# SmallVCM/SmallVCM

Hardware: AMD Instinct MI355X
Metric: Mpaths/sec (light+camera), VCM scene 1 at 2048^2 (higher is better)
Workload: dtype f32; 1 GPU; scene 1 -a vcm 2048x2048 maxPathLength 10 minPathLength 0 radiusFactor 0.003 radiusAlpha 0.75 seed 1234, iterations 5..408 timed; parallelism=1 renderer(s) (iteration-parallel, smallvcm.cxx:61-108) on one GPU, 1 in flight

## Files before the change

### smallvcm_amd/csrc/vcm_api.hip

```cpp
#include <hip/hip_runtime.h>
#include <stdio.h>
#include <stdlib.h>
#include <string.h>
#include <string>
#include <new>
#include <mutex>
#include <vector>
#include <condition_variable>
#include <atomic>

#include "vcm_kernels.h"
#include "vcm_kat.h"
#include "scene_host.h"
#include "scene_kind.h"
#include "vcm_denoise.h"
#include "vcm_variance.h"
#include "vcm_robust.h"
#include "vcm_parts.h"
#include "vcm_display.h"

using namespace vcm;

static thread_local std::string g_err;
static int fail(const char *what, const char *detail)
// ... 70 lines not shown
    Arena *arenas[VCM_MAX_ARENAS];
};
static std::atomic<unsigned long long> g_threadCounter{0};
static thread_local unsigned long long g_threadId = 0;
static unsigned long long this_thread_id() { if (!g_threadId) g_threadId = ++g_threadCounter; return g_threadId; }

#ifndef VCM_MERGE_DEFAULT
#define VCM_MERGE_DEFAULT VCM_MERGE_PAIRS
#endif
struct vcm_ctx : Scratch {
    SceneHost *scene;
    bool useVM, useVC, lightTraceOnly, ppm;
    int renderer;
    float baseRadius, radiusAlpha;
    int seed, device, rank, world;
    int resX, resY, N, p0, nLocal;
    int iterations;

    hipStream_t stream;
    bool ownStream;
    hipStream_t side;
    hipEvent_t evFork, evBbox, evGrid;
    bool gridInFlight;
    hipStream_t splat;
    hipEvent_t evSplatFork, evSplatDone;
    hipEvent_t evSortFork, evSorted;
    hipEvent_t evZero;
    bool prezeroed, sortInFlight;
    bool splatInFlight;
    bool resolveInFlight;
    hipEvent_t evMergeDone, evSplatWork, evResolved;
    hipEvent_t evPreMerge;
    bool mergeInFlight;
    bool deviceReady;
    ArenaPool *pool;
    Arena *arena; bool holdsArena;

    DScene *dScene;
    char *dSceneBlob;
    float *dFb;
    unsigned char *dRngLight, *dRngCam;
    GridHeader *dHdr;
    unsigned long long *dStats;
    unsigned long long *dStatsRing;
    unsigned long long *dStamps;
    float radiusRing[VCM_STAMP_RING];
// ... 240 lines not shown
}
static void arena_release(vcm_ctx *c, bool recordEvent)
{
    if (!c->holdsArena) return;
    Arena *a = c->arena;
    const bool recorded = recordEvent && a->eventReady && hipEventRecord(a->lastUse, c->resolveInFlight ? c->splat : c->stream) == hipSuccess;
    c->holdsArena = false;
    {
        std::lock_guard<std::mutex> g(*a->mtx);
        if (recorded) { a->lastValid = true; a->lastUser = c; }
        a->busy = false;
        a->ownerThread = 0;
    }
    a->cv->notify_all();
}
static int abort_iteration(vcm_ctx *c, int rc)
{
    if (rc != 0 && c && c->inIteration && c->holdsArena) {
        const std::string keep = g_err;
        (void)hipStreamSynchronize(c->stream);
        if (c->deviceReady) { (void)hipStreamSynchronize(c->side); (void)hipStreamSynchronize(c->splat); }
        c->mergeInFlight = false;
        c->gridInFlight = false;
        c->splatInFlight = false;
        c->resolveInFlight = false;
        c->sortInFlight = false;
        c->inIteration = false;
        arena_release(c, false);
        g_err = keep;
    } else if (rc != 0 && c && c->holdsArena && !c->inIteration) {
        arena_release(c, false);
    }
    return rc;
}

static int scratch_readable(vcm_ctx *c, const char *what)
{
    if (!c || !c->deviceReady || (!c->inIteration && c->iterations == 0)) return fail(what, "no iteration has run");
    if (!c->holdsArena) {
        if (!c->arena) return fail(what, "no iteration has run");
        std::lock_guard<std::mutex> g(*c->arena->mtx);
        if (c->arena->lastUser != c)
            return fail(what, "the iteration scratch has since been used by another context of this device");
    }
    return 0;
}
// ... 179 lines not shown
    hipLaunchKernelGGL((k_scan_apply<T>), dim3(nTiles), dim3(VCM_SCAN_BLOCK), 0, stream, in, n, (const int *)tileSums, out, totalOut, writeTotalAtN);
    HIPCHK(hipGetLastError());
    return 0;
}
template <typename T>
static int launch_scan(vcm_ctx *c, const T *in, int n, int *out, int *totalOut, int writeTotalAtN)
{
    return launch_scan_on<T>(c, 0, c->stream, in, n, out, totalOut, writeTotalAtN, take_stamps(c, c->stream));
}

static int shape_knob(const char *key)
{
    static const char *spec = getenv("SMALLVCM_AMD_SHAPE");
    if (!spec) return 0;
    const size_t n = strlen(key);
    for (const char *p = spec; *p;) {
        if (!strncmp(p, key, n) && p[n] == '=') { const int v = atoi(p + n + 1); return v > 0 ? v : 0; }
        const char *q = strchr(p, ',');
        if (!q) break;
        p = q + 1;
    }
    return 0;
}
static void trace_launch_shape(int nLocal, int *blocks, int *chunk, bool lightPass = false)
{
    int waves = (nLocal + VCM_WAVE - 1) / VCM_WAVE;
    const int tw = shape_knob("trace_waves");
    int maxWaves = tw ? tw : 256 * 16;
    if (!tw && nLocal <= (1 << 20)) maxWaves = 256 * 12;
    const int lw = shape_knob("light_waves");
    if (lightPass && lw) maxWaves = lw;
    if (maxWaves > VCM_MAX_TRACE_WAVES) maxWaves = VCM_MAX_TRACE_WAVES;
    if (waves > maxWaves) waves = maxWaves;
    if (waves < 1) waves = 1;
    const int wavesPerBlock = VCM_TRACE_BLOCK / VCM_WAVE;
    *blocks = (waves + wavesPerBlock - 1) / wavesPerBlock;
    const int totalWaves = *blocks * wavesPerBlock;
    int ch = nLocal / totalWaves;
    const int ce = shape_knob("trace_chunk");
    if (ce) ch = ce;
    if (!ce && !tw && nLocal <= (1 << 20)) {
        ch = 128;
        const int need = (nLocal + ch - 1) / ch;
        if (totalWaves > need) *blocks = (need + wavesPerBlock - 1) / wavesPerBlock;
    }
    *chunk = ch < 64 ? 64 : (ch > 256 && !ce ? 256 : ch);
}


template <class Launch>
static int read_back(vcm_ctx *c, const char *who, size_t bytes, void *host, Launch &&launch)
{
// ... 381 lines not shown
    P.wavefront = vcm_is_wavefront(c, maxLen);
    P.renderer = c->renderer;
    P.iteration = iteration;
    const bool big = c->nLocal >= (1 << 20);
    P.qblockVertex = big ? 512 : 256; P.qblockDI = big ? 512 : 256; P.qblockVC = big ? 1024 : 512;
    {
        const int perPath = shape_knob("buckets_per_path");
        const int per = perPath ? perPath : (c->nLocal > (1 << 20) ? 16 : 4);
        long long nb = (long long)per * c->nLocal;
        if (nb < (1 << 18)) nb = 1 << 18;
        P.nBuckets = nb < VCM_QSORT_BUCKETS ? (int)nb : VCM_QSORT_BUCKETS;
    }
    P.foreignOut = 0;

    c->nPend[0] = c->nPend[1] = 0;
    if (mark(c, EV_START)) return -1;
    c->dStats = c->dStatsRing + (size_t)(c->iterations % VCM_STAMP_RING) * VCM_STAT_SLOTS;
    c->radiusRing[c->iterations % VCM_STAMP_RING] = radius;
    if (zero_ranges(c->stream, c->dStats, VCM_STAT_SLOTS * sizeof(unsigned long long), c->store.count, (size_t)c->nLocal ,
                    c->vs.count, 32 * sizeof(int) ,
                    c->dHdr, 6 * sizeof(uint32_t) )) return -1;
    c->importedRecords = false;
    c->importedSorted = false;
    c->gridBuilt = c->cameraTraced = c->merged = c->splatsPending = c->recordsValid = c->countedInCamera = c->scatteredInDI = c->gridInFlight = c->splatInFlight = c->bboxPreset = c->bboxFromLight = c->bboxFinal = c->prezeroed = c->sortInFlight = c->spaceSet = c->mergeImported = false;
    c->splatInFlight = c->resolveInFlight;
    c->inIteration = true;
    c->lastMergeKernel = 0;
    c->evValid = false;
    return 0;
}

static int task_blocks(int nLocal)
{
    const int n = shape_knob("task_blocks");
    if (n) return n;
    if (nLocal >= (1 << 21)) return 256 * 12;
    const int b = nLocal / 1024;
    return b < 512 ? 512 : (b > 1024 ? 1024 : b);
}
static int merge_blocks(int nLocal, int N)
{
    const int n = shape_knob("merge_blocks") >= 8 ? (shape_knob("merge_blocks") & ~7) : 0;
    if (n) return n;
    if (nLocal >= (1 << 21)) return 16384;
    int b = (nLocal / 1024) & ~7;
    b = b < 512 ? 512 : (b > 2048 ? 2048 : b);
    if (N >= (1 << 21) && nLocal < N) { const long long d = (16384ll * nLocal / N) & ~7ll; if (d > b) b = (int)d; }
// ... 112 lines not shown
        launch_kind<kWrapLens | kWrapPick | kWrapSobol | kWrapGgx>(c, [&](auto tag) {
            using S = typename decltype(tag)::type;
            hipLaunchKernelGGL((k_light_trace<0, S>), dim3(blocks), dim3(VCM_TRACE_BLOCK), 0, c->stream, c->dScene, c->P, c->store,
                               c->dFb, c->dRngLight, c->dStats, chunk, take_stamps(c, c->stream), c->vs.count + 16, c->dHdr);
        });
    HIPCHK(hipGetLastError());
    c->bboxFromLight = c->world == 1;
    if (mark(c, EV_LIGHT_K1)) return -1;
    if (launch_scan<unsigned char>(c, c->store.count, c->nLocal, c->dPathStart, c->dLocalTotal, 0)) return -1;
    if (c->mergeInFlight) { HIPCHK(hipStreamWaitEvent(c->stream, c->evMergeDone, 0)); c->mergeInFlight = false; }
    bool countsSet = false;
    if (c->useVM || wf) {
        c->recordsValid = c->useVM && c->world > 1 && !c->sortedExchange;
        const bool fold = c->world == 1;
        hipLaunchKernelGGL((c->ggx ? k_compact_records_ggx : k_compact_records), dim3(aux_blocks(c->nLocal)), dim3(256), 0, c->stream, (const DScene *)c->dScene, c->P, c->store, c->dPathStart,
                           c->dRecordsLocal, c->dSlotOfVertex, c->recordsValid ? 1 : 0, fold ? c->dHdr : (GridHeader *)NULL,
                           (const int *)c->dLocalTotal, (fold && c->bboxFromLight) ? 1 : 0);
        HIPCHK(hipGetLastError());
        countsSet = fold;
        if (fold && c->bboxFromLight) c->bboxFinal = true;
    }
    if (wf && (c->useVC || c->lightTraceOnly)) {
        c->splatsPending = true;
        if (c->world == 1 && flush_light_splats(c)) return -1;
    }
    if (mark(c, EV_LIGHT)) return -1;
    if (!countsSet) {
        hipLaunchKernelGGL(k_set_counts, dim3(1), dim3(1), 0, c->stream, c->dHdr, c->dLocalTotal, 1, 0, take_stamps(c, c->stream));
        HIPCHK(hipGetLastError());
    }
    return 0;
}

static int ensure_records(vcm_ctx *c)
{
    if (c->recordsValid || !c->useVM) return 0;
    hipLaunchKernelGGL((c->ggx ? k_compact_records_ggx : k_compact_records), dim3(aux_blocks(c->nLocal)), dim3(256), 0, c->stream, (const DScene *)c->dScene, c->P, c->store, c->dPathStart,
                       c->dRecordsLocal, c->dSlotOfVertex, 1, (GridHeader *)NULL, (const int *)c->dLocalTotal, 0);
    HIPCHK(hipGetLastError());
    c->recordsValid = true;
    return 0;
}

int vcm_light_records(vcm_ctx *c, void **devPtr, long long *count)
{
    if (scratch_readable(c, "vcm_light_records")) return -1;
    if (use_device(c)) return -1;
// ... 78 lines not shown

static int vcm_import_light_records_impl(vcm_ctx *c, const void *devPtr, const long long *counts, int nSeg, long long strideRecords)
{
    if (!c || !c->inIteration) return fail("vcm_import_light_records", "no iteration in progress");
    if (c->world <= 1 || !c->dRecordsAll) return fail("vcm_import_light_records", "context is not sharded");
    if (use_device(c)) return -1;
    long long total = 0;
    const size_t recBytes = VCM_MERGE_RECORD_FLOATS * sizeof(float);
    for (int s = 0; s < nSeg; s++) {
        if (counts[s] < 0) return fail("vcm_import_light_records", "negative count");
        if (total + counts[s] > (long long)c->arena->capS * (long long)c->arena->capN) return fail("vcm_import_light_records", "too many records");
        if (counts[s] > 0)
            HIPCHK(hipMemcpyAsync((char *)c->dRecordsAll + (size_t)total * recBytes,
                                  (const char *)devPtr + (size_t)s * (size_t)strideRecords * recBytes,
                                  (size_t)counts[s] * recBytes, hipMemcpyDeviceToDevice, c->stream));
        total += counts[s];
    }
    hipLaunchKernelGGL(k_set_counts, dim3(1), dim3(1), 0, c->stream, c->dHdr, c->dLocalTotal, 0, (int)total, take_stamps(c, c->stream));
    HIPCHK(hipGetLastError());
    c->importedRecords = true;
    return 0;
}

static const I2 *sort_cells_radix(vcm_ctx *c, hipStream_t q, int scanSlot, const VertexSource &recs)
{
    const int nCells = c->P.nCells;
    int bits = 1;
    while (bits < 31 && (1ll << bits) < (long long)nCells) bits++;
    const int passes = (bits + 7) / 8;
    const int V = radix_sort_blocks(c->nLocal);
    static_assert(256 * VCM_RSORT_MAX_BLOCKS <= VCM_QSORT_BUCKETS, "the scan scratch (dTileSums) is sized for the bucket table: the digit matrix must not be larger");
    const StampArgs none = { { NULL, NULL, NULL, NULL } };
    uint32_t *key[2] = { (uint32_t *)c->dCellId, (uint32_t *)c->dSortedIndex };
    I2 *pay[2] = { (I2 *)c->dUnsorted, (I2 *)c->dUnsorted + (size_t)c->arena->capS * c->arena->capN };
    int *hist = c->dRadixHist, *scanned = c->dRadixHist + 256 * VCM_RSORT_MAX_BLOCKS;
    hipLaunchKernelGGL(k_cell_keys, dim3(V), dim3(256), 0, q, c->P, recs, (const GridHeader *)c->dHdr, key[0], pay[0], hist, take_stamps(c, q));
    int cur = 0;
    for (int p = 0; p < passes; p++) {
        if (p > 0) hipLaunchKernelGGL(k_radix_hist, dim3(V), dim3(256), 0, q, (const uint32_t *)key[cur], (const GridHeader *)c->dHdr, 8 * p, hist);
        if (hipGetLastError() != hipSuccess) { fail("vcm_build_grid", "radix histogram launch"); return NULL; }
        if (launch_scan_on<int>(c, scanSlot, q, hist, 256 * V, scanned, NULL, 0, none)) return NULL;
        hipLaunchKernelGGL(k_radix_scatter, dim3(V), dim3(256), 0, q, (const uint32_t *)key[cur], (const I2 *)pay[cur], key[cur ^ 1], pay[cur ^ 1],
                           (const GridHeader *)c->dHdr, 8 * p, (const int *)scanned);
        cur ^= 1;
    }
    hipLaunchKernelGGL(k_cell_starts, dim3(aux_blocks(c->nLocal)), dim3(256), 0, q, (const uint32_t *)key[cur], (const GridHeader *)c->dHdr, nCells, c->dCellStart);
    if (hipGetLastError() != hipSuccess) { fail("vcm_build_grid", "radix sort launch"); return NULL; }
    return pay[cur];
}

static int sorted_shape(vcm_ctx *c, long long strideRecords, int *K, int *nBlocks, long long *slabWords, const char *who)
{
    if (!c) return fail(who, "ctx is NULL");
    if (c->world <= 1) return fail(who, "the context is not sharded");
    if (!c->useVM) return fail(who, "the algorithm does not merge: nothing to exchange");
    if (c->world > VCM_SORTED_MAX_SHARDS) return fail(who, "more than 64 shards: use the unsorted exchange");
    if (strideRecords < 1 || strideRecords >= (1ll << 24)) return fail(who, "1 <= records per shard < 2^24 (the index shares a word with the path length): use the unsorted exchange");
    *K = sorted_block_cells(c->world);
    *nBlocks = (c->N + *K - 1) / *K;
    const long long w = strideRecords * VCM_SORTED_WORDS + (long long)*nBlocks + 1;
    *slabWords = (w + 3) & ~3ll;
    return 0;
}
extern "C" long long vcm_sorted_slab_words(vcm_ctx *c, long long strideRecords)
{
    int K, nBlocks; long long words;
    if (sorted_shape(c, strideRecords, &K, &nBlocks, &words, "vcm_sorted_slab_words")) return -1;
    return words;
}
// ... 40 lines not shown
    long long total = 0;
    for (int s = 0; s < nSeg; s++) {
        if (counts[s] < 0 || counts[s] > strideRecords) return fail("vcm_import_sorted_light_records", "a count exceeds the slab");
        in.rankBase[s] = (int)total;
        total += counts[s];
    }
    in.rankBase[nSeg] = (int)total;
    if (total > (long long)c->arena->capS * (long long)c->arena->capN) return fail("vcm_import_sorted_light_records", "too many records");
    hipLaunchKernelGGL(k_set_counts, dim3(1), dim3(1), 0, c->stream, c->dHdr, c->dLocalTotal, 0, (int)total, take_stamps(c, c->stream));
    HIPCHK(hipGetLastError());
    c->importedSorted = true;
    c->importedRecords = false;
    return 0;
}
extern "C" int vcm_sort_light_records(vcm_ctx *c, void *dstDev, long long strideRecords)
{
    return abort_iteration(c, vcm_sort_light_records_impl(c, dstDev, strideRecords));
}
extern "C" int vcm_import_sorted_light_records(vcm_ctx *c, const void *gathered, const long long *counts, int nSeg, long long strideRecords)
{
    return abort_iteration(c, vcm_import_sorted_light_records_impl(c, gathered, counts, nSeg, strideRecords));
}

static int join_grid(vcm_ctx *c)
{
    if (!c->gridInFlight) return 0;
    HIPCHK(hipStreamWaitEvent(c->stream, c->evGrid, 0));
    c->gridInFlight = false;
    return 0;
}

static int vcm_build_grid_impl(vcm_ctx *c)
{
    if (!c || !c->inIteration) return fail("vcm_build_grid", "no iteration in progress");
    if (use_device(c)) return -1;
    if (flush_light_splats(c)) return -1;
    c->gridBuilt = true;
    if (c->useVM) {
        hipStream_t q = c->side;
        HIPCHK(hipEventRecord(c->evFork, c->stream));
        HIPCHK(hipStreamWaitEvent(q, c->evFork, 0));
        if (mark_on(c, EV_GRID_K0, q)) return -1;
        if (c->importedSorted) {
            if (!c->bboxPreset) return fail("vcm_build_grid", "sorted records without the box they were sorted with");
            const int blocks = c->sortedIn.nBlocks < 8192 ? c->sortedIn.nBlocks : 8192;
            hipLaunchKernelGGL(k_grid_merge_blocks, dim3(blocks), dim3(256), 0, q, c->P, (const GridHeader *)c->dHdr, c->sortedIn, c->dCellStart,
                               c->dGx, c->dGy, c->dGz, c->dGb, c->dG1, c->dG2, c->dG3, c->dSortedIndex, take_stamps(c, q));
            HIPCHK(hipGetLastError());
            if (mark_on(c, EV_GRID, q)) return -1;
            hipLaunchKernelGGL(k_note_grid_vertices, dim3(1), dim3(1), 0, q, (const GridHeader *)c->dHdr, c->dStats + STAT_COUNT, take_stamps(c, q));
            HIPCHK(hipGetLastError());
            HIPCHK(hipEventRecord(c->evGrid, q));
            c->gridInFlight = true;
            if (!c->P.wavefront && join_grid(c)) return -1;
            return 0;
        }
        VertexSource recs;
        recs.records = c->importedRecords ? c->dRecordsAll : (c->recordsValid ? c->dRecordsLocal : NULL);
        recs.store = c->store;
        recs.slotOfVertex = c->dSlotOfVertex;
        const int nCells = c->P.nCells;
        const dim3 g(aux_blocks(c->nLocal)), b(256);
        const bool radix = grid_sort_is_radix(c);
        if (c->prezeroed) HIPCHK(hipStreamWaitEvent(q, c->evZero, 0));
        else if (!radix && zero_ranges(q, c->dCellCount, ((size_t)nCells + 1) * sizeof(int))) return -1;
        bool boxOnSide = false;
        if (!c->bboxPreset) {
            if (c->bboxFromLight && !recs.records) {
                if (!c->bboxFinal) { hipLaunchKernelGGL(k_bbox_finalize, dim3(1), dim3(64), 0, q, c->dHdr, 1); boxOnSide = true; }
            } else {
                boxOnSide = true;
                hipLaunchKernelGGL(k_grid_init, dim3(1), dim3(64), 0, q, c->dHdr, take_stamps(c, q));
                hipLaunchKernelGGL(k_bbox, dim3(512), b, 0, q, recs, c->dHdr);
                hipLaunchKernelGGL(k_bbox_finalize, dim3(1), dim3(64), 0, q, c->dHdr, 0);
            }
        }
        HIPCHK(hipEventRecord(c->evBbox, q));
        const I2 *sorted = NULL;
        if (radix) {
            if (!(sorted = sort_cells_radix(c, q, 1, recs))) return -1;
        } else {
            hipLaunchKernelGGL(k_cell_count, g, b, 0, q, c->P, recs, (const GridHeader *)c->dHdr, c->dCellId,
                               c->dSortedIndex , c->dCellCount, take_stamps(c, q));
            HIPCHK(hipGetLastError());
            if (launch_scan_on<int>(c, 1, q, c->dCellCount, nCells, c->dCellStart, NULL, 1, take_stamps(c, q))) return -1;
            hipLaunchKernelGGL(k_cell_scatter, g, b, 0, q, (const GridHeader *)c->dHdr, (const int *)c->dCellId,
                               (const int *)c->dSortedIndex, (const int *)c->dCellStart,
                               recs.records ? (const int *)NULL : (const int *)c->dSlotOfVertex, c->dUnsorted);
        }
        hipLaunchKernelGGL((c->ggx ? k_cell_rank_gather_ggx : k_cell_rank_gather), g, b, 0, q, (const DScene *)c->dScene, (const GridHeader *)c->dHdr, recs,
                           (const int *)c->dCellStart, (const I4 *)c->dUnsorted, sorted, c->dGx,
                           c->dGy, c->dGz, c->dGb, c->dG1, c->dG2, c->dG3, c->dSortedIndex);
        if (mark_on(c, EV_GRID, q)) return -1;
        hipLaunchKernelGGL(k_note_grid_vertices, dim3(1), dim3(1), 0, q, (const GridHeader *)c->dHdr, c->dStats + STAT_COUNT, take_stamps(c, q));
        HIPCHK(hipGetLastError());
        HIPCHK(hipEventRecord(c->evGrid, q));
        if (boxOnSide) HIPCHK(hipStreamWaitEvent(c->stream, c->evBbox, 0));
        c->gridInFlight = true;
        if (!c->P.wavefront && join_grid(c)) return -1;
    } else {
        if (mark(c, EV_GRID_K0)) return -1;
        if (mark(c, EV_GRID)) return -1;
    }
    return 0;
}

static GridStore grid_of(vcm_ctx *c)
{
    GridStore grid;
    grid.cellStart = c->dCellStart; grid.gx = c->dGx; grid.gy = c->dGy; grid.gz = c->dGz; grid.gb = c->dGb; grid.g1 = c->dG1; grid.g2 = c->dG2; grid.g3 = c->dG3;
    grid.hdr = c->dHdr;
    return grid;
}

static int vcm_trace_camera_impl(vcm_ctx *c)
{
    if (!c || !c->inIteration) return fail("vcm_trace_camera", "no iteration in progress");
    if (use_device(c)) return -1;
    if (flush_light_splats(c)) return -1;
    c->cameraTraced = true;
    if (c->lightTraceOnly) return 0;
    int blocks, chunk;
    trace_launch_shape(c->nLocal, &blocks, &chunk);
    if (c->resolveInFlight) HIPCHK(hipStreamWaitEvent(c->stream, c->evResolved, 0));
    if (mark(c, EV_CAMERA_K0)) return -1;
    if (c->renderer) {
        if (c->renderer == 1)
            launch_kind<kWrapLens | kWrapPick | kWrapSobol | kWrapGgx>(c, [&](auto tag) {
                using S = typename decltype(tag)::type;
                hipLaunchKernelGGL((k_path_trace<S>), dim3(blocks), dim3(VCM_TRACE_BLOCK), 0, c->stream, c->dScene, c->P, c->dCamOut,
                                   c->dRngCam, c->dStats, chunk, take_stamps(c, c->stream), c->vs.count + 8);
            });
        else
            launch_kind<kWrapLens | kWrapSobol>(c, [&](auto tag) {
                using S = typename decltype(tag)::type;
                hipLaunchKernelGGL((k_eye_light<S>), dim3(2048), dim3(256), 0, c->stream, c->dScene, c->P, c->dCamOut, c->dRngCam,
                                   c->dStats, take_stamps(c, c->stream));
            });
        HIPCHK(hipGetLastError());
        if (mark(c, EV_CAMERA_K1)) return -1;
        if (mark(c, EV_CONNECT_K1)) return -1;
        return 0;
    }
    if (c->P.wavefront) {
        c->countedInCamera = c->useVM && (c->gridBuilt || c->bboxPreset);
        c->vs.sortHdr = c->countedInCamera ? c->dHdr : NULL;
// ... 5 lines not shown
            else if (zero_ranges(c->stream, c->dQueryCount, ((size_t)c->P.nBuckets + 1) * sizeof(int))) return -1;
        }
        launch_kind<kWrapLens | kWrapPick | kWrapSobol | kWrapGgx>(c, [&](auto tag) {
            using S = typename decltype(tag)::type;
            hipLaunchKernelGGL((k_camera_trace<1, S>), dim3(blocks), dim3(VCM_TRACE_BLOCK), 0, c->stream, c->dScene, c->P,
                               c->store, grid_of(c), c->vs, c->dCamOut, c->dCamMask, c->dRngCam, c->dStats, chunk, take_stamps(c, c->stream));
        });
        if (mark(c, EV_CAMERA_K1)) return -1;
        if (c->useVC) {
            c->scatteredInDI = c->countedInCamera && c->P.minLen <= 2;
            const bool inlineSort = c->scatteredInDI && (c->nLocal <= (1 << 20) || grid_sort_is_radix(c));
            if (c->countedInCamera && c->world == 1 && !inlineSort) {
                HIPCHK(hipEventRecord(c->evSortFork, c->stream));
                HIPCHK(hipStreamWaitEvent(c->side, c->evSortFork, 0));
                const StampArgs none = { { NULL, NULL, NULL, NULL } };
                if (launch_scan_on<int>(c, 3, c->side, c->dQueryCount, c->P.nBuckets, c->dQueryStart, NULL, 1, none)) return -1;
                hipLaunchKernelGGL(k_query_scatter, dim3(aux_blocks(c->nLocal)), dim3(256), 0, c->side, c->vs, (const int *)c->dQueryKey,
                                   (const int *)c->dQueryArrival, (const int *)c->dQueryStart, c->dSortedVertex);
                HIPCHK(hipEventRecord(c->evSorted, c->side));
                c->sortInFlight = true;
                c->scatteredInDI = false;
            }
            if (c->scatteredInDI && launch_scan<int>(c, c->dQueryCount, c->P.nBuckets, c->dQueryStart, NULL, 1)) return -1;
            {
                HIPCHK(hipEventRecord(c->evSplatFork, c->stream));
                HIPCHK(hipStreamWaitEvent(c->splat, c->evSplatFork, 0));
                launch_kind<kWrapGgx>(c, [&](auto tag) {
                    using S = typename decltype(tag)::type;
                    hipLaunchKernelGGL((k_connect_vc<S>), dim3(task_blocks(c->nLocal)), dim3(VCM_TASK_BLOCK), 0, c->splat, c->dScene, c->P, c->vs,
                                       c->store, c->dStats);
                });
                HIPCHK(hipEventRecord(c->evSplatDone, c->splat));
                c->splatInFlight = true;
            }
            launch_kind<kWrapPick | kWrapSobol | kWrapGgx>(c, [&](auto tag) {
                using S = typename decltype(tag)::type;
                hipLaunchKernelGGL((k_connect_di<S>), dim3(task_blocks(c->nLocal)), dim3(VCM_TASK_BLOCK), 0, c->stream, c->dScene, c->P, c->vs,
                                   c->dStats, c->scatteredInDI ? (const int *)c->dQueryStart : (const int *)NULL,
                                   c->scatteredInDI ? c->dSortedVertex : (int *)NULL, take_stamps(c, c->stream));
            });
        }
        if (mark(c, EV_CONNECT_K1)) return -1;
    } else {
        if (c->useVM && !c->gridBuilt) return fail("vcm_trace_camera", "strict mode merges inside the camera pass: call vcm_build_grid first");
        launch_kind<kWrapLens | kWrapPick | kWrapSobol | kWrapGgx>(c, [&](auto tag) {
            using S = typename decltype(tag)::type;
            hipLaunchKernelGGL((k_camera_trace<0, S>), dim3(blocks), dim3(VCM_TRACE_BLOCK), 0, c->stream, c->dScene, c->P,
                               c->store, grid_of(c), c->vs, c->dCamOut, c->dCamMask, c->dRngCam, c->dStats, chunk, take_stamps(c, c->stream));
        });
        if (mark(c, EV_CAMERA_K1)) return -1;
        if (mark(c, EV_CONNECT_K1)) return -1;
    }
    HIPCHK(hipGetLastError());
    if (c->world > 1 && flush_stamps(c, c->stream)) return -1;
    return 0;
}

#define VCM_SPACE_BLOCKS 512
static int space_scratch(vcm_ctx *c)
{
    if (c->dSpaceMatrix) return 0;
    HIPCHK(hipMalloc((void **)&c->dSpaceMatrix, sizeof(int) * VCM_SPACE_MAX_SLABS * VCM_SPACE_BLOCKS));
    HIPCHK(hipMalloc((void **)&c->dSpaceScanned, sizeof(int) * (VCM_SPACE_MAX_SLABS * VCM_SPACE_BLOCKS + 1)));
    HIPCHK(hipMalloc((void **)&c->dSpaceTotals, sizeof(int) * VCM_SPACE_MAX_SLABS));
    HIPCHK(hipMalloc((void **)&c->dSpaceHist, sizeof(int) * 256));
    return 0;
}
static int space_ready(vcm_ctx *c, const char *who)
{
    if (!c || !c->inIteration) return fail(who, "no iteration in progress");
    if (c->world <= 1) return fail(who, "the context is not sharded");
    if (!c->useVM || !c->P.wavefront) return fail(who, "needs a merging algorithm in wavefront mode");
    if (use_device(c)) return -1;
    return space_scratch(c);
}
static int vcm_space_histogram_impl(vcm_ctx *c, int axis, float *lo, float *binWidth, int *hist256)
// ... 152 lines not shown
    if (!c->lightTraceOnly) {
        bool mergeAside = false;
        if (mark(c, EV_MERGE_K0)) return -1;
        if (c->P.wavefront && c->useVM && c->mergeImported) {
            if (mark(c, EV_SORT_K1)) return -1;
        } else if (c->P.wavefront && c->useVM) {
            if (!c->gridBuilt) return fail("vcm_merge", "call vcm_build_grid first");
            const int nb = c->P.nBuckets;
            if (!c->countedInCamera) {
                if (c->prezeroed) HIPCHK(hipStreamWaitEvent(c->stream, c->evZero, 0));
                if (zero_ranges(c->stream, c->dQueryCount, ((size_t)nb + 1) * sizeof(int))) return -1;
                hipLaunchKernelGGL(k_query_count, dim3(aux_blocks(c->nLocal)), dim3(256), 0, c->stream, c->P, c->vs,
                                   (const GridHeader *)c->dHdr, c->dQueryKey, c->dQueryArrival, c->dQueryCount, take_stamps(c, c->stream));
            }
            if (c->sortInFlight) {
                HIPCHK(hipStreamWaitEvent(c->stream, c->evSorted, 0));
                c->sortInFlight = false;
            } else if (!c->scatteredInDI) {
                if (launch_scan<int>(c, c->dQueryCount, nb, c->dQueryStart, NULL, 1)) return -1;
                hipLaunchKernelGGL(k_query_scatter, dim3(aux_blocks(c->nLocal)), dim3(256), 0, c->stream, c->vs, (const int *)c->dQueryKey,
                                   (const int *)c->dQueryArrival, (const int *)c->dQueryStart, c->dSortedVertex);
            }
            if (mark(c, EV_SORT_K1)) return -1;
            if (c->gridInFlight && hipEventQuery(c->evGrid) != hipSuccess) { (void)hipGetLastError(); if (flush_stamps(c, c->stream)) return -1; }
            if (join_grid(c)) return -1;
            mergeAside = (c->nLocal <= (1 << 20) || !c->useVC) && c->world == 1 && !c->strictOrder;
            hipStream_t ks = c->stream;
            if (mergeAside) {
                if (flush_stamps(c, c->stream)) return -1;
                HIPCHK(hipEventRecord(c->evPreMerge, c->stream));
                HIPCHK(hipStreamWaitEvent(c->side, c->evPreMerge, 0));
                ks = c->side;
            }
            static int mergeChunk = 0;
            if (!mergeChunk) mergeChunk = shape_knob("merge_chunk") ? shape_knob("merge_chunk") : 16;
            int mergeStaged = c->mergeKind;
            if (mergeStaged == VCM_MERGE_PAIRS && (int)c->scene->materials.size() > VCM_PAIR_MATERIALS) mergeStaged = VCM_MERGE_WALK;
            c->lastMergeKernel = mergeStaged;
            hipLaunchKernelGGL(merge_kernel(mergeStaged, c->intPhong, c->ggx), dim3(merge_blocks(c->nLocal, c->N)), dim3(VCM_MERGE_BLOCK), 0, ks, c->dScene, c->P, grid_of(c),
                               c->vs, (const int *)c->dSortedVertex, (const int *)(c->dQueryStart + nb), c->dStats, mergeChunk, take_stamps(c, c->stream));
        } else {
            if (mark(c, EV_SORT_K1)) return -1;
        }
        if (mergeAside) {
            HIPCHK(hipGetLastError());
            HIPCHK(hipEventRecord(c->evMergeDone, c->side));
// ... 1173 lines not shown
```

### smallvcm_amd/csrc/vcm_kernels.h

```cpp
#ifndef SMALLVCM_AMD_VCM_KERNELS_H
#define SMALLVCM_AMD_VCM_KERNELS_H

#include <hip/hip_runtime.h>
#include "vcm_core.h"

namespace vcm {

enum { STAT_LIGHT_RAYS = 0, STAT_CAMERA_RAYS, STAT_SHADOW_RAYS, STAT_MERGE_QUERIES, STAT_MERGE_CANDIDATES,
       STAT_MERGE_ACCEPTED, STAT_CONNECTIONS, STAT_LIGHT_SPLATS, STAT_STORED, STAT_COUNT };

#define VCM_TRACE_BLOCK 256
#define VCM_WAVE 64

struct StampArgs { unsigned long long *p[4]; };
__device__ __forceinline__ void stamp_entry(const StampArgs &s)
{
    if (blockIdx.x == 0 && threadIdx.x == 0 && s.p[0]) {
        const unsigned long long t = wall_clock64();
#pragma unroll
        for (int k = 0; k < 4; k++) if (s.p[k]) *s.p[k] = t;
    }
}

__device__ __forceinline__ unsigned lane_id() { return __builtin_amdgcn_mbcnt_hi(~0u, __builtin_amdgcn_mbcnt_lo(~0u, 0u)); }
// ... 1626 lines not shown
            for (int round = 0; round < VCM_RSORT_TILE / 256; round++) {
                if (validBits & (1u << round)) {
                    const uint32_t d = (k[round] >> shift) & 255u;
                    const int pos = sRun[w][d] + r[round];
                    sKey[pos] = k[round];
                    sPay[pos] = p[round];
                }
            }
            __syncthreads();
            for (int j = tid; j < m; j += 256) {
                const uint32_t kk = sKey[j];
                const uint32_t d = (kk >> shift) & 255u;
                const int dst = sGlobal[d] + (j - sBinStart[d]);
                keyOut[dst] = kk;
                payOut[dst] = sPay[j];
            }
            __syncthreads();
            sGlobal[tid] += total;
        }
    }
#endif
}

__global__ void __launch_bounds__(256) k_cell_starts(const uint32_t *__restrict__ key, const GridHeader *__restrict__ hdr, int nCells, int *cellStart)
{
#if defined(__HIP_DEVICE_COMPILE__)
    const int n = hdr->nRecords;
    const int lane = (int)threadIdx.x & 63;
    const int stride = (int)(gridDim.x * blockDim.x);
    for (int base = (int)(blockIdx.x * blockDim.x) + ((int)threadIdx.x & ~63); base <= n; base += stride) {
        const int pos = base + lane;
        int c0 = 0, len = 0;
        if (pos <= n) {
            const int prev = pos > 0 ? (int)key[pos - 1] : -1;
            const int cur = pos < n ? (int)key[pos] : nCells;
            c0 = prev + 1; len = cur - prev;
        }
        const int head = len < 8 ? len : 8;
        for (int c = 0; c < head; c++) cellStart[c0 + c] = pos;
        unsigned long long longOnes = __ballot(len > 8);
        while (longOnes) {
            const int l = __ffsll((long long)longOnes) - 1;
            longOnes &= longOnes - 1ull;
            const int s = __shfl(c0 + 8, l, 64), e = __shfl(c0 + len, l, 64), v = __shfl(pos, l, 64);
            for (int c = s + lane; c < e; c += 64) cellStart[c] = v;
        }
    }
#endif
}

template <class S>
__device__ __forceinline__ void cell_rank_gather_body(const DScene *__restrict__ scp, const GridHeader *__restrict__ hdr, const VertexSource &src,
                                                      const int *__restrict__ cellStart, const I4 *__restrict__ unsorted, const I2 *__restrict__ sorted,
                                                      float *gx, float *gy, float *gz, float *gb, F4 *g1, F4 *g2, F2 *g3, int *sortedIndex)
{
    const int n = hdr->nRecords;
    for (int pos = blockIdx.x * blockDim.x + threadIdx.x; pos < n; pos += gridDim.x * blockDim.x) {
        I4 me;
        int dst = pos;
        if (sorted) {
            const I2 e = sorted[pos];
            me.x = e.x; me.y = e.y; me.z = 0; me.w = 0;
        } else {
            me = unsorted[pos];
            const int cell = me.z;
            const int lo = cellStart[cell], hi = cellStart[cell + 1];
            int rank = 0;
            for (int q = lo; q < hi; q++) rank += (unsorted[q].x < me.x) ? 1 : 0;
            dst = lo + rank;
        }
        const int i = me.x;
        F2 t;
        if (src.records) {
            const float *r = src.records + (size_t)i * VCM_MERGE_RECORD_FLOATS;
            gx[dst] = r[0]; gy[dst] = r[1]; gz[dst] = r[2];
            gb[grid_blocked_index(dst, 0)] = r[0]; gb[grid_blocked_index(dst, 1)] = r[1]; gb[grid_blocked_index(dst, 2)] = r[2];
            g1[dst] = mk4(r[3], r[4], r[5], r[11]);
            g2[dst] = mk4(r[6], r[7], r[8], r[9]);
            t.x = r[10]; t.y = r[12];
        } else {
            const size_t slot = (size_t)me.y;
            const F4 a = lv(src.store, slot, 0), b = lv(src.store, slot, 1), d = lv(src.store, slot, 3);
            const F4 e = light_vertex_wdir_contprob(*static_cast<const S *>(scp), a, lv(src.store, slot, 2), d, false);
            gx[dst] = a.x; gy[dst] = a.y; gz[dst] = a.z;
            gb[grid_blocked_index(dst, 0)] = a.x; gb[grid_blocked_index(dst, 1)] = a.y; gb[grid_blocked_index(dst, 2)] = a.z;
            g1[dst] = e;
            g2[dst] = b;
            t.x = d.w; t.y = u2f(f2u(a.w) & 0xffu);
        }
        g3[dst] = t;
        if (sortedIndex) sortedIndex[dst] = i;
    }
}
__global__ void __launch_bounds__(256) k_cell_rank_gather(const DScene *__restrict__ scp, const GridHeader *__restrict__ hdr, VertexSource src,
                                   const int *__restrict__ cellStart, const I4 *__restrict__ unsorted, const I2 *__restrict__ sorted,
                                   float *gx, float *gy, float *gz, float *gb, F4 *g1, F4 *g2, F2 *g3, int *sortedIndex)
{
    const int n = hdr->nRecords;
    for (int pos = blockIdx.x * blockDim.x + threadIdx.x; pos < n; pos += gridDim.x * blockDim.x) {
        I4 me;
        int dst = pos;
        if (sorted) {
            const I2 e = sorted[pos];
            me.x = e.x; me.y = e.y; me.z = 0; me.w = 0;
        } else {
            me = unsorted[pos];
            const int cell = me.z;
            const int lo = cellStart[cell], hi = cellStart[cell + 1];
            int rank = 0;
            for (int q = lo; q < hi; q++) rank += (unsorted[q].x < me.x) ? 1 : 0;
            dst = lo + rank;
        }
        const int i = me.x;
        F2 t;
        if (src.records) {
            const float *r = src.records + (size_t)i * VCM_MERGE_RECORD_FLOATS;
            gx[dst] = r[0]; gy[dst] = r[1]; gz[dst] = r[2];
            gb[grid_blocked_index(dst, 0)] = r[0]; gb[grid_blocked_index(dst, 1)] = r[1]; gb[grid_blocked_index(dst, 2)] = r[2];
            g1[dst] = mk4(r[3], r[4], r[5], r[11]);
            g2[dst] = mk4(r[6], r[7], r[8], r[9]);
            t.x = r[10]; t.y = r[12];
        } else {
            const size_t slot = (size_t)me.y;
            const F4 a = lv(src.store, slot, 0), b = lv(src.store, slot, 1), d = lv(src.store, slot, 3);
            const F4 e = light_vertex_wdir_contprob(*scp, a, lv(src.store, slot, 2), d, false);
            gx[dst] = a.x; gy[dst] = a.y; gz[dst] = a.z;
            gb[grid_blocked_index(dst, 0)] = a.x; gb[grid_blocked_index(dst, 1)] = a.y; gb[grid_blocked_index(dst, 2)] = a.z;
            g1[dst] = e;
            g2[dst] = b;
            t.x = d.w; t.y = u2f(f2u(a.w) & 0xffu);
        }
        g3[dst] = t;
        if (sortedIndex) sortedIndex[dst] = i;
    }
}
__global__ void __launch_bounds__(256) k_cell_rank_gather_ggx(const DScene *__restrict__ scp, const GridHeader *__restrict__ hdr, VertexSource src,
                                       const int *__restrict__ cellStart, const I4 *__restrict__ unsorted, const I2 *__restrict__ sorted,
                                       float *gx, float *gy, float *gz, float *gb, F4 *g1, F4 *g2, F2 *g3, int *sortedIndex)
{
    cell_rank_gather_body<WithGgx<DScene>>(scp, hdr, src, cellStart, unsorted, sorted, gx, gy, gz, gb, g1, g2, g3, sortedIndex);
}


#define VCM_SORTED_WORDS 13
#define VCM_SORTED_MAX_SHARDS 64
#define VCM_SORTED_MAX_TABLE 4096
inline __host__ __device__ int sorted_block_cells(int S)
{
    const int k = VCM_SORTED_MAX_TABLE / (S > 0 ? S : 1);
    int p = 16;
    while (p * 2 <= k && p < 1024) p *= 2;
    return p;
}

template <class S>
__device__ __forceinline__ void cell_rank_pack_body(const DScene *__restrict__ scp, const GridHeader *__restrict__ hdr, const VertexSource &src,
                                                    const int *__restrict__ cellStart, const I4 *__restrict__ unsorted, const I2 *__restrict__ sorted,
                                                    uint32_t *slab, int *blockStart, int nCells, int K, int nBlocks)
{
    const int n = hdr->nRecords;
    for (int b = blockIdx.x * blockDim.x + threadIdx.x; b <= nBlocks; b += gridDim.x * blockDim.x) {
        const long long c = (long long)b * K;
        blockStart[b] = cellStart[c < nCells ? (int)c : nCells];
// ... 173 lines not shown
```

Baseline: 1254 Mpaths/s.

## Defer grid gather tail and fuse cell-start computation into rank gather kernel

Adds an 'early plan' for large single-GPU VCM runs. The grid is built before the light splats are flushed, and the final gather/cell-starts step is deferred so it can run on the side stream behind the camera trace. The cell_starts kernel and the note_grid_vertices kernel are fused into the rank-gather kernel, which removes two launches. The camera trace uses fewer waves in this mode to leave room for the overlapped work. The cost is more complex stream ordering and the risk of contention between the overlapped kernels.

```diff
diff --git a/smallvcm_amd/csrc/vcm_api.hip b/smallvcm_amd/csrc/vcm_api.hip
--- a/smallvcm_amd/csrc/vcm_api.hip
+++ b/smallvcm_amd/csrc/vcm_api.hip
@@ -116,6 +116,8 @@
     hipStream_t side;
     hipEvent_t evFork, evBbox, evGrid;
     bool gridInFlight;
+    bool gridTailPending;
+    VertexSource tailRecs; const I2 *tailSorted; const uint32_t *tailKey;
     hipStream_t splat;
     hipEvent_t evSplatFork, evSplatDone;
     hipEvent_t evSortFork, evSorted;
@@ -402,6 +404,7 @@
         if (c->deviceReady) { (void)hipStreamSynchronize(c->side); (void)hipStreamSynchronize(c->splat); }
         c->mergeInFlight = false;
         c->gridInFlight = false;
+        c->gridTailPending = false;
         c->splatInFlight = false;
         c->resolveInFlight = false;
         c->sortInFlight = false;
@@ -627,12 +630,37 @@
     }
     return 0;
 }
-static void trace_launch_shape(int nLocal, int *blocks, int *chunk, bool lightPass = false)
+static bool shape_word(const char *key, const char *word)
+{
+    static const char *spec = getenv("SMALLVCM_AMD_SHAPE");
+    if (!spec) return false;
+    const size_t n = strlen(key), m = strlen(word);
+    for (const char *p = spec; *p;) {
+        if (!strncmp(p, key, n) && p[n] == '=') return !strncmp(p + n + 1, word, m) && (p[n + 1 + m] == ',' || p[n + 1 + m] == 0);
+        const char *q = strchr(p, ',');
+        if (!q) break;
+        p = q + 1;
+    }
+    return false;
+}
+static int plan_forced()
+{
+    static const int f = shape_word("plan", "early") ? 1 : (shape_word("plan", "late") ? 2 : 0);
+    return f;
+}
+static bool plan_early(const vcm_ctx *c)
+{
+    if (c->world != 1 || c->strictOrder) return false;
+    if (plan_forced()) return plan_forced() == 1;
+    return c->useVC && c->useVM && c->nLocal > (1 << 20);
+}
+static void trace_launch_shape(int nLocal, int *blocks, int *chunk, bool lightPass = false, bool early = false)
 {
     int waves = (nLocal + VCM_WAVE - 1) / VCM_WAVE;
     const int tw = shape_knob("trace_waves");
     int maxWaves = tw ? tw : 256 * 16;
     if (!tw && nLocal <= (1 << 20)) maxWaves = 256 * 12;
+    if (!tw && early && !lightPass && nLocal > (1 << 20)) maxWaves = 256 * 12;
     const int lw = shape_knob("light_waves");
     if (lightPass && lw) maxWaves = lw;
     if (maxWaves > VCM_MAX_TRACE_WAVES) maxWaves = VCM_MAX_TRACE_WAVES;
@@ -1060,7 +1088,7 @@
                     c->dHdr, 6 * sizeof(uint32_t) )) return -1;
     c->importedRecords = false;
     c->importedSorted = false;
-    c->gridBuilt = c->cameraTraced = c->merged = c->splatsPending = c->recordsValid = c->countedInCamera = c->scatteredInDI = c->gridInFlight = c->splatInFlight = c->bboxPreset = c->bboxFromLight = c->bboxFinal = c->prezeroed = c->sortInFlight = c->spaceSet = c->mergeImported = false;
+    c->gridBuilt = c->cameraTraced = c->merged = c->splatsPending = c->recordsValid = c->countedInCamera = c->scatteredInDI = c->gridInFlight = c->gridTailPending = c->splatInFlight = c->bboxPreset = c->bboxFromLight = c->bboxFinal = c->prezeroed = c->sortInFlight = c->spaceSet = c->mergeImported = false;
     c->splatInFlight = c->resolveInFlight;
     c->inIteration = true;
     c->lastMergeKernel = 0;
@@ -1219,7 +1247,7 @@
     }
     if (wf && (c->useVC || c->lightTraceOnly)) {
         c->splatsPending = true;
-        if (c->world == 1 && flush_light_splats(c)) return -1;
+        if (c->world == 1 && !(c->useVM && plan_early(c)) && flush_light_splats(c)) return -1;
     }
     if (mark(c, EV_LIGHT)) return -1;
     if (!countsSet) {
@@ -1344,7 +1372,7 @@
     return 0;
 }
 
-static const I2 *sort_cells_radix(vcm_ctx *c, hipStream_t q, int scanSlot, const VertexSource &recs)
+static const I2 *sort_cells_radix(vcm_ctx *c, hipStream_t q, int scanSlot, const VertexSource &recs, const uint32_t **sortedKey = NULL)
 {
     const int nCells = c->P.nCells;
     int bits = 1;
@@ -1356,8 +1384,8 @@
     uint32_t *key[2] = { (uint32_t *)c->dCellId, (uint32_t *)c->dSortedIndex };
     I2 *pay[2] = { (I2 *)c->dUnsorted, (I2 *)c->dUnsorted + (size_t)c->arena->capS * c->arena->capN };
     int *hist = c->dRadixHist, *scanned = c->dRadixHist + 256 * VCM_RSORT_MAX_BLOCKS;
-    hipLaunchKernelGGL(k_cell_keys, dim3(V), dim3(256), 0, q, c->P, recs, (const GridHeader *)c->dHdr, key[0], pay[0], hist, take_stamps(c, q));
-    int cur = 0;
+    int cur = passes & 1;
+    hipLaunchKernelGGL(k_cell_keys, dim3(V), dim3(256), 0, q, c->P, recs, (const GridHeader *)c->dHdr, key[cur], pay[cur], hist, take_stamps(c, q));
     for (int p = 0; p < passes; p++) {
         if (p > 0) hipLaunchKernelGGL(k_radix_hist, dim3(V), dim3(256), 0, q, (const uint32_t *)key[cur], (const GridHeader *)c->dHdr, 8 * p, hist);
         if (hipGetLastError() != hipSuccess) { fail("vcm_build_grid", "radix histogram launch"); return NULL; }
@@ -1366,7 +1394,8 @@
                            (const GridHeader *)c->dHdr, 8 * p, (const int *)scanned);
         cur ^= 1;
     }
-    hipLaunchKernelGGL(k_cell_starts, dim3(aux_blocks(c->nLocal)), dim3(256), 0, q, (const uint32_t *)key[cur], (const GridHeader *)c->dHdr, nCells, c->dCellStart);
+    if (sortedKey) *sortedKey = key[cur];
+    else hipLaunchKernelGGL(k_cell_starts, dim3(aux_blocks(c->nLocal)), dim3(256), 0, q, (const uint32_t *)key[cur], (const GridHeader *)c->dHdr, nCells, c->dCellStart);
     if (hipGetLastError() != hipSuccess) { fail("vcm_build_grid", "radix sort launch"); return NULL; }
     return pay[cur];
 }
@@ -1453,8 +1482,25 @@
     return abort_iteration(c, vcm_import_sorted_light_records_impl(c, gathered, counts, nSeg, strideRecords));
 }
 
+static int finish_grid_build(vcm_ctx *c, bool behindMain)
+{
+    hipStream_t q = c->side;
+    c->gridTailPending = false;
+    if (behindMain) {
+        HIPCHK(hipEventRecord(c->evSortFork, c->stream));
+        HIPCHK(hipStreamWaitEvent(q, c->evSortFork, 0));
+    }
+    hipLaunchKernelGGL((c->ggx ? k_cell_rank_gather_ggx : k_cell_rank_gather), dim3(aux_blocks(c->nLocal)), dim3(256), 0, q, (const DScene *)c->dScene,
+                       (const GridHeader *)c->dHdr, c->tailRecs, c->dCellStart, (const I4 *)c->dUnsorted, c->tailSorted, c->dGx,
+                       c->dGy, c->dGz, c->dGb, c->dG1, c->dG2, c->dG3, c->dSortedIndex, c->tailKey, c->P.nCells, c->dStats + STAT_COUNT);
+    HIPCHK(hipGetLastError());
+    HIPCHK(hipEventRecord(c->evGrid, q));
+    if (mark_on(c, EV_GRID, q)) return -1;
+    return flush_stamps(c, q);
+}
 static int join_grid(vcm_ctx *c)
 {
+    if (c->gridTailPending && finish_grid_build(c, false)) return -1;
     if (!c->gridInFlight) return 0;
     HIPCHK(hipStreamWaitEvent(c->stream, c->evGrid, 0));
     c->gridInFlight = false;
@@ -1465,7 +1511,8 @@
 {
     if (!c || !c->inIteration) return fail("vcm_build_grid", "no iteration in progress");
     if (use_device(c)) return -1;
-    if (flush_light_splats(c)) return -1;
+    const bool gridFirst = c->useVM && !c->importedSorted && plan_early(c);
+    if (!gridFirst && flush_light_splats(c)) return -1;
     c->gridBuilt = true;
     if (c->useVM) {
         hipStream_t q = c->side;
@@ -1508,8 +1555,9 @@
         }
         HIPCHK(hipEventRecord(c->evBbox, q));
         const I2 *sorted = NULL;
+        const uint32_t *sortedKey = NULL;
         if (radix) {
-            if (!(sorted = sort_cells_radix(c, q, 1, recs))) return -1;
+            if (!(sorted = sort_cells_radix(c, q, 1, recs, &sortedKey))) return -1;
         } else {
             hipLaunchKernelGGL(k_cell_count, g, b, 0, q, c->P, recs, (const GridHeader *)c->dHdr, c->dCellId,
                                c->dSortedIndex , c->dCellCount, take_stamps(c, q));
@@ -1519,15 +1567,13 @@
                                (const int *)c->dSortedIndex, (const int *)c->dCellStart,
                                recs.records ? (const int *)NULL : (const int *)c->dSlotOfVertex, c->dUnsorted);
         }
-        hipLaunchKernelGGL((c->ggx ? k_cell_rank_gather_ggx : k_cell_rank_gather), g, b, 0, q, (const DScene *)c->dScene, (const GridHeader *)c->dHdr, recs,
-                           (const int *)c->dCellStart, (const I4 *)c->dUnsorted, sorted, c->dGx,
-                           c->dGy, c->dGz, c->dGb, c->dG1, c->dG2, c->dG3, c->dSortedIndex);
-        if (mark_on(c, EV_GRID, q)) return -1;
-        hipLaunchKernelGGL(k_note_grid_vertices, dim3(1), dim3(1), 0, q, (const GridHeader *)c->dHdr, c->dStats + STAT_COUNT, take_stamps(c, q));
         HIPCHK(hipGetLastError());
-        HIPCHK(hipEventRecord(c->evGrid, q));
+        c->tailRecs = recs; c->tailSorted = sorted; c->tailKey = sortedKey;
+        c->gridTailPending = gridFirst && radix && c->P.wavefront && c->useVC && c->P.minLen <= 2 && !c->cameraTraced;
+        if (!c->gridTailPending && finish_grid_build(c, false)) return -1;
         if (boxOnSide) HIPCHK(hipStreamWaitEvent(c->stream, c->evBbox, 0));
         c->gridInFlight = true;
+        if (gridFirst && flush_light_splats(c)) return -1;
         if (!c->P.wavefront && join_grid(c)) return -1;
     } else {
         if (mark(c, EV_GRID_K0)) return -1;
@@ -1552,7 +1598,7 @@
     c->cameraTraced = true;
     if (c->lightTraceOnly) return 0;
     int blocks, chunk;
-    trace_launch_shape(c->nLocal, &blocks, &chunk);
+    trace_launch_shape(c->nLocal, &blocks, &chunk, false, plan_early(c));
     if (c->resolveInFlight) HIPCHK(hipStreamWaitEvent(c->stream, c->evResolved, 0));
     if (mark(c, EV_CAMERA_K0)) return -1;
     if (c->renderer) {
@@ -1604,6 +1650,7 @@
                 c->scatteredInDI = false;
             }
             if (c->scatteredInDI && launch_scan<int>(c, c->dQueryCount, c->P.nBuckets, c->dQueryStart, NULL, 1)) return -1;
+            if (c->gridTailPending && finish_grid_build(c, c->scatteredInDI)) return -1;
             {
                 HIPCHK(hipEventRecord(c->evSplatFork, c->stream));
                 HIPCHK(hipStreamWaitEvent(c->splat, c->evSplatFork, 0));
@@ -1634,6 +1681,7 @@
         if (mark(c, EV_CONNECT_K1)) return -1;
     }
     HIPCHK(hipGetLastError());
+    if (c->gridTailPending && finish_grid_build(c, false)) return -1;
     if (c->world > 1 && flush_stamps(c, c->stream)) return -1;
     return 0;
 }
@@ -1832,6 +1880,7 @@
                                    (const int *)c->dQueryArrival, (const int *)c->dQueryStart, c->dSortedVertex);
             }
             if (mark(c, EV_SORT_K1)) return -1;
+            if (c->gridTailPending && finish_grid_build(c, false)) return -1;
             if (c->gridInFlight && hipEventQuery(c->evGrid) != hipSuccess) { (void)hipGetLastError(); if (flush_stamps(c, c->stream)) return -1; }
             if (join_grid(c)) return -1;
             mergeAside = (c->nLocal <= (1 << 20) || !c->useVC) && c->world == 1 && !c->strictOrder;
diff --git a/smallvcm_amd/csrc/vcm_kernels.h b/smallvcm_amd/csrc/vcm_kernels.h
--- a/smallvcm_amd/csrc/vcm_kernels.h
+++ b/smallvcm_amd/csrc/vcm_kernels.h
@@ -1672,40 +1672,49 @@
 #endif
 }
 
+__device__ __forceinline__ void cell_starts_wave(const uint32_t *__restrict__ key, int n, int nCells, int pos, int lane, int *cellStart)
+{
+#if defined(__HIP_DEVICE_COMPILE__)
+    int c0 = 0, len = 0;
+    if (pos <= n) {
+        const int prev = pos > 0 ? (int)key[pos - 1] : -1;
+        const int cur = pos < n ? (int)key[pos] : nCells;
+        c0 = prev + 1; len = cur - prev;
+    }
+    const int head = len < 8 ? len : 8;
+    for (int c = 0; c < head; c++) cellStart[c0 + c] = pos;
+    unsigned long long longOnes = __ballot(len > 8);
+    while (longOnes) {
+        const int l = __ffsll((long long)longOnes) - 1;
+        longOnes &= longOnes - 1ull;
+        const int s = __shfl(c0 + 8, l, 64), e = __shfl(c0 + len, l, 64), v = __shfl(pos, l, 64);
+        for (int c = s + lane; c < e; c += 64) cellStart[c] = v;
+    }
+#endif
+}
 __global__ void __launch_bounds__(256) k_cell_starts(const uint32_t *__restrict__ key, const GridHeader *__restrict__ hdr, int nCells, int *cellStart)
 {
-#if defined(__HIP_DEVICE_COMPILE__)
     const int n = hdr->nRecords;
     const int lane = (int)threadIdx.x & 63;
     const int stride = (int)(gridDim.x * blockDim.x);
+    for (int base = (int)(blockIdx.x * blockDim.x) + ((int)threadIdx.x & ~63); base <= n; base += stride)
+        cell_starts_wave(key, n, nCells, base + lane, lane, cellStart);
+}
+
+template <class S>
+__device__ __forceinline__ void cell_rank_gather_body(const DScene *__restrict__ scp, const GridHeader *__restrict__ hdr, const VertexSource &src,
+                                                      int *cellStart, const I4 *__restrict__ unsorted, const I2 *__restrict__ sorted,
+                                                      float *gx, float *gy, float *gz, float *gb, F4 *g1, F4 *g2, F2 *g3, int *sortedIndex,
+                                                      const uint32_t *__restrict__ sortedKey, int nCells, unsigned long long *note)
+{
+    const int n = hdr->nRecords;
+    const int lane = (int)threadIdx.x & 63;
+    const int stride = (int)(gridDim.x * blockDim.x);
+    if (note && blockIdx.x == 0 && threadIdx.x == 0) *note = (unsigned long long)n;
     for (int base = (int)(blockIdx.x * blockDim.x) + ((int)threadIdx.x & ~63); base <= n; base += stride) {
         const int pos = base + lane;
-        int c0 = 0, len = 0;
-        if (pos <= n) {
-            const int prev = pos > 0 ? (int)key[pos - 1] : -1;
-            const int cur = pos < n ? (int)key[pos] : nCells;
-            c0 = prev + 1; len = cur - prev;
-        }
-        const int head = len < 8 ? len : 8;
-        for (int c = 0; c < head; c++) cellStart[c0 + c] = pos;
-        unsigned long long longOnes = __ballot(len > 8);
-        while (longOnes) {
-            const int l = __ffsll((long long)longOnes) - 1;
-            longOnes &= longOnes - 1ull;
-            const int s = __shfl(c0 + 8, l, 64), e = __shfl(c0 + len, l, 64), v = __shfl(pos, l, 64);
-            for (int c = s + lane; c < e; c += 64) cellStart[c] = v;
-        }
-    }
-#endif
-}
-
-template <class S>
-__device__ __forceinline__ void cell_rank_gather_body(const DScene *__restrict__ scp, const GridHeader *__restrict__ hdr, const VertexSource &src,
-                                                      const int *__restrict__ cellStart, const I4 *__restrict__ unsorted, const I2 *__restrict__ sorted,
-                                                      float *gx, float *gy, float *gz, float *gb, F4 *g1, F4 *g2, F2 *g3, int *sortedIndex)
-{
-    const int n = hdr->nRecords;
-    for (int pos = blockIdx.x * blockDim.x + threadIdx.x; pos < n; pos += gridDim.x * blockDim.x) {
+        if (sortedKey) cell_starts_wave(sortedKey, n, nCells, pos, lane, cellStart);
+        if (pos >= n) continue;
         I4 me;
         int dst = pos;
         if (sorted) {
@@ -1743,11 +1752,18 @@
     }
 }
 __global__ void __launch_bounds__(256) k_cell_rank_gather(const DScene *__restrict__ scp, const GridHeader *__restrict__ hdr, VertexSource src,
-                                   const int *__restrict__ cellStart, const I4 *__restrict__ unsorted, const I2 *__restrict__ sorted,
-                                   float *gx, float *gy, float *gz, float *gb, F4 *g1, F4 *g2, F2 *g3, int *sortedIndex)
+                                   int *cellStart, const I4 *__restrict__ unsorted, const I2 *__restrict__ sorted,
+                                   float *gx, float *gy, float *gz, float *gb, F4 *g1, F4 *g2, F2 *g3, int *sortedIndex,
+                                   const uint32_t *__restrict__ sortedKey, int nCells, unsigned long long *note)
 {
     const int n = hdr->nRecords;
-    for (int pos = blockIdx.x * blockDim.x + threadIdx.x; pos < n; pos += gridDim.x * blockDim.x) {
+    const int lane = (int)threadIdx.x & 63;
+    const int stride = (int)(gridDim.x * blockDim.x);
+    if (note && blockIdx.x == 0 && threadIdx.x == 0) *note = (unsigned long long)n;
+    for (int base = (int)(blockIdx.x * blockDim.x) + ((int)threadIdx.x & ~63); base <= n; base += stride) {
+        const int pos = base + lane;
+        if (sortedKey) cell_starts_wave(sortedKey, n, nCells, pos, lane, cellStart);
+        if (pos >= n) continue;
         I4 me;
         int dst = pos;
         if (sorted) {
@@ -1785,10 +1801,11 @@
     }
 }
 __global__ void __launch_bounds__(256) k_cell_rank_gather_ggx(const DScene *__restrict__ scp, const GridHeader *__restrict__ hdr, VertexSource src,
-                                       const int *__restrict__ cellStart, const I4 *__restrict__ unsorted, const I2 *__restrict__ sorted,
-                                       float *gx, float *gy, float *gz, float *gb, F4 *g1, F4 *g2, F2 *g3, int *sortedIndex)
-{
-    cell_rank_gather_body<WithGgx<DScene>>(scp, hdr, src, cellStart, unsorted, sorted, gx, gy, gz, gb, g1, g2, g3, sortedIndex);
+                                       int *cellStart, const I4 *__restrict__ unsorted, const I2 *__restrict__ sorted,
+                                       float *gx, float *gy, float *gz, float *gb, F4 *g1, F4 *g2, F2 *g3, int *sortedIndex,
+                                       const uint32_t *__restrict__ sortedKey, int nCells, unsigned long long *note)
+{
+    cell_rank_gather_body<WithGgx<DScene>>(scp, hdr, src, cellStart, unsorted, sorted, gx, gy, gz, gb, g1, g2, g3, sortedIndex, sortedKey, nCells, note);
 }
 
 
```

Result: no change. 1253 Mpaths/s, median of 2 (-0.1%).
